# SonyCSLParis/vqcpc-bach

Measured on AMD Instinct MI355X. Metric: encoder-train windows/sec (Bach 4-voice, seq=256), higher is better.
Workload: dtype f32

## Files before the change

### include/vqcpc.h

```cpp
#ifndef VQCPC_H
#define VQCPC_H

#include <stdint.h>

#ifdef __cplusplus
extern "C" {
#endif

#define VQCPC_ABI_VERSION 2

#define VQCPC_OK 0
#define VQCPC_EINVAL (-1)
#define VQCPC_ELAUNCH (-2)
#define VQCPC_EWORKSPACE (-3)

int vqcpc_abi_version(void);
const char* vqcpc_last_error(void);
int vqcpc_clear_runtime_error(void);

int vqcpc_dropout_mask(float* mask, int64_t n, float p, uint64_t seed, void* stream);

int vqcpc_check_tokens(const int64_t* tokens, int64_t n, int n_voices, const int32_t* limits, int64_t* clamped, int32_t* flag,
                       void* stream);

// ... 147 lines not shown
                            const float* mean, const float* rstd, float* d_s, float* d_r, float* d_gamma, float* d_beta,
                            int64_t M, int d, float drop_p, uint64_t seed, void* workspace, int64_t workspace_bytes,
                            void* stream);
int vqcpc_add_layernorm_fwd_b16(const float* x, int64_t ldx, const float* r, const float* gamma, const float* beta, float* y,
                                void* y_bf16, float* mean, float* rstd, int64_t M, int d, float eps, float drop_p,
                                uint64_t seed, void* stream);
int vqcpc_add_layernorm_bwd_b16(const float* dy, const float* x, int64_t ldx, const float* r, const float* gamma,
                                const float* mean, const float* rstd, float* d_s, float* d_r, void* d_r_bf16, float* d_gamma,
                                float* d_beta, int64_t M, int d, float drop_p, uint64_t seed, void* workspace,
                                int64_t workspace_bytes, void* stream);
int vqcpc_layernorm_fwd_xb16(const void* x_bf16, int64_t ldx, const float* gamma, const float* beta, float* y, void* y_bf16,
                             float* mean, float* rstd, int64_t M, int d, float eps, void* stream);
int vqcpc_layernorm_bwd_xb16(const float* dy, const void* x_bf16, int64_t ldx, const float* gamma, const float* mean,
                             const float* rstd, float* d_s, void* d_s_bf16, float* d_r, void* d_r_bf16, float* d_gamma,
                             float* d_beta, int64_t M, int d, float drop_p, uint64_t seed, void* workspace,
                             int64_t workspace_bytes, void* stream);
int vqcpc_layernorm_bwd_b16io(const void* dy_bf16, const void* x_bf16, int64_t ldx, const float* gamma, const float* mean,
                              const float* rstd, float* d_s, void* d_s_bf16, float* d_r, void* d_r_bf16, float* d_gamma,
                              float* d_beta, int64_t M, int d, float drop_p, uint64_t seed, void* workspace,
                              int64_t workspace_bytes, void* stream);
int vqcpc_add_layernorm_bwd_partials(int64_t M, int d, int has_r);
int vqcpc_reduce_grouped(int n, const void* const* ws, const int64_t* stride, const int* nsplit, void* const* out,
                         const int64_t* count, int accumulate, void* stream);

int vqcpc_vq_fwd(const float* z, const float* codebooks, int64_t R, int ncb, int K, int dsub, float beta, int squared,
                 int assign, int64_t* idx, float* zq_sg, float* loss, void* stream);
int64_t vqcpc_vq_bwd_workspace(int64_t R, int ncb, int K, int dsub);
int vqcpc_vq_bwd(const float* z, const float* codebooks, const int64_t* idx, const float* g_zq, const float* g_loss,
                 int64_t R, int ncb, int K, int dsub, float beta, int squared, float* d_z, float* d_codebooks,
                 void* workspace, int64_t workspace_bytes, void* stream);

int64_t vqcpc_vq_ema_stats_workspace(int64_t R, int ncb, int K, int dsub);
int vqcpc_vq_ema_stats(const float* z, const int64_t* idx, int64_t R, int ncb, int K, int dsub, float* stats, void* workspace,
                       int64_t workspace_bytes, void* stream);
int vqcpc_vq_commit_bwd(const float* z, const float* codebooks, const int64_t* idx, const float* g_zq, const float* g_loss,
                        int64_t R, int ncb, int K, int dsub, float beta, int squared, float* d_z, void* stream);
int vqcpc_vq_ema_update(const float* stats, float* cluster_size, float* ema_sum, float* codebooks, int ncb, int K, int dsub,
                        float g, float h, float eps, void* stream);

int vqcpc_vq_restart_candidates(const float* z, int64_t R, int ncb, int K, int dsub, uint64_t seed, uint64_t step,
                                const uint64_t* step_dev, int rank, int world, float* cand, void* stream);
int vqcpc_vq_ema_restart(const float* cand, float* cluster_size, float* ema_sum, float* codebooks, int ncb, int K, int dsub,
                         float thr, int32_t* restarts, void* stream);

int vqcpc_dropout_selu_fwd(const float* h, float* out, int64_t n, float drop_p, uint64_t seed, void* stream);
int vqcpc_dropout_selu_bwd(const float* h, const float* g_out, float* g_h, int64_t n, float drop_p, uint64_t seed,
// ... 231 lines not shown
```

### vqcpc_bach_amd/csrc/common.h

```cpp
#pragma once
#include <stdlib.h>
#include <hip/hip_runtime.h>
#include <stdint.h>
#include <stdio.h>

#include "../../include/vqcpc.h"

namespace vq {

void set_error(const char* fmt, ...);

#define VQ_REQUIRE(cond, ...)                   \
    do {                                        \
        if (!(cond)) {                          \
            vq::set_error(__VA_ARGS__);         \
            return VQCPC_EINVAL;                \
        }                                       \
    } while (0)

#define VQ_CHECK_LAUNCH(name)                                                        \
    do {                                                                             \
        hipError_t e_ = hipGetLastError();                                           \
        if (e_ != hipSuccess) {                                                      \
            vq::set_error("%s: launch failed: %s", name, hipGetErrorString(e_));     \
// ... 43 lines not shown
__device__ __forceinline__ uint32_t rng_u24(uint64_t seed, uint64_t idx) {
    const uint64_t se = rng_seed_eff(seed);
    return rng_u24_from_x0(rng_x0(se, static_cast<uint32_t>(idx)), static_cast<uint32_t>(se >> 32));
}
__host__ __device__ __forceinline__ uint32_t drop_threshold(float p) { return static_cast<uint32_t>(p * 16777216.0f); }
__device__ __forceinline__ float drop_scale(uint64_t seed, uint64_t idx, uint32_t thr, float inv_keep) {
    if (thr == 0) return 1.0f;
    return rng_u24(seed, idx) >= thr ? inv_keep : 0.0f;
}

__device__ __forceinline__ float wave_sum(float v) {
#pragma unroll
    for (int o = 32; o > 0; o >>= 1) v += __shfl_xor(v, o, 64);
    return v;
}
__device__ __forceinline__ float wave_max(float v) {
#pragma unroll
    for (int o = 32; o > 0; o >>= 1) v = fmaxf(v, __shfl_xor(v, o, 64));
    return v;
}

int launch_reduce_splits(const float* ws, int64_t stride, int nsplit, float* out, int64_t count, int accumulate,
                         hipStream_t stream);
int launch_reduce_splits2(const float* ws, int64_t stride, int nsplit, float* out, int64_t count, const float* ws2,
                          int64_t stride2, float* out2, int64_t count2, int accumulate, hipStream_t stream);

#ifdef __HIPCC__
typedef float vq_f32x2_t __attribute__((ext_vector_type(2)));
typedef __bf16 vq_bf16x2_t __attribute__((ext_vector_type(2)));
__device__ __forceinline__ uint32_t bf16x2_rn(float e0, float e1) {
    const vq_f32x2_t v = {e0, e1};
    return __builtin_bit_cast(uint32_t, __builtin_convertvector(v, vq_bf16x2_t));
}
__device__ __forceinline__ void store4_out(float* __restrict__ base, int64_t off, float a, float b, float c, float d, int out16) {
    if (out16)
        *reinterpret_cast<uint2*>(reinterpret_cast<unsigned short*>(base) + off) = make_uint2(bf16x2_rn(a, b), bf16x2_rn(c, d));
    else
        *reinterpret_cast<float4*>(base + off) = make_float4(a, b, c, d);
}
__device__ __forceinline__ void store1_out(float* __restrict__ base, int64_t off, float a, int out16) {
    if (out16) reinterpret_cast<unsigned short*>(base)[off] = (unsigned short)(bf16x2_rn(a, 0.0f) & 0xFFFFu);
    else base[off] = a;
}
#endif

int64_t relattn16_bwd_workspace(int64_t n_blocks, int H, int hd);
// ... 8 lines not shown
```

### vqcpc_bach_amd/csrc/relattn.hip

```cpp
#include "common.h"
#include "relattn_forms.h"
#include <stdlib.h>

namespace vq {

constexpr int kAttThreads = 256;
constexpr int kPad = 4;

template <int L, int HD>
struct AttCfg {
    static constexpr int LPP = 4 * L;
    static constexpr int PPW = 64 / LPP;
    static constexpr int SLOTS = 4 * PPW;
    static constexpr int JPL = L / 4;
    static constexpr int CPL = HD / 4;
    static constexpr int RS = HD + kPad;
    static constexpr int NE = 2 * L - 1;
    static constexpr int FWD_FLOATS = (3 * L + NE) * RS + L * (L + 1);
    static constexpr int BWD_FLOATS = (4 * L + NE) * RS + 2 * L * (L + 1);
};

template <int L, int HD>
__device__ __forceinline__ void stage_rows(float* dst, const float* __restrict__ src, int64_t ld, int sl, float mul,
                                           const int64_t* __restrict__ tok = nullptr) {
// ... 317 lines not shown
#pragma unroll
                            for (int c4 = 0; c4 < C::CPL / 4; ++c4) {
                                const float4 q = *reinterpret_cast<const float4*>(Qs + ii * C::RS + jg * C::CPL + c4 * 4);
                                de[a][c4 * 4 + 0] += ds * q.x; de[a][c4 * 4 + 1] += ds * q.y;
                                de[a][c4 * 4 + 2] += ds * q.z; de[a][c4 * 4 + 3] += ds * q.w;
                            }
                        }
                    }
                }
            }
        }
    }
    float* dst = ws + ((((int64_t)blockIdx.x * NS + nsub) * H + h) * C::NE) * HD;
#pragma unroll
    for (int a = 0; a < 2; ++a) {
        const int r = i + a * L;
        if (r < C::NE) {
#pragma unroll
            for (int c = 0; c < C::CPL; ++c) dst[r * HD + jg * C::CPL + c] = de[a][c];
        }
    }
}

__global__ __launch_bounds__(256) void relattn_de_split(const float* __restrict__ tot, int H, int L, int HD,
                                                        float* __restrict__ d_e1, float* __restrict__ d_e2) {
    const int NE = 2 * L - 1;
    const int o = blockIdx.x * blockDim.x + threadIdx.x;
    if (o >= H * NE * HD) return;
    const int c = o % HD, r = (o / HD) % NE, h = o / (HD * NE);
    const float acc = tot[o];
    if (r < L) d_e1[((int64_t)h * L + r) * HD + c] = acc;
    else d_e2[((int64_t)h * L + (r - L + 1)) * HD + c] = acc;
    if (r == 0) d_e2[((int64_t)h * L) * HD + c] = 0.0f;
}

static int att_blocks_per_wg(int64_t n_blocks, int slots, int H) {
    const int ns = std::max(1, slots / H);
    int64_t b = ceil_div(n_blocks, 2048);
    b = round_up(std::max<int64_t>(b, ns), ns);
    return (int)b;
}

template <int L, int HD>
static int launch_fwd(const float* qkv, int64_t ldq, const float* e1, const float* e2, float* ctx, int64_t ldo,
                      float* probs, int64_t n_blocks, int H, float drop_p, uint64_t seed, hipStream_t s,
                      const int64_t* tokens, int o16) {
    using C = AttCfg<L, HD>;
    const size_t lds = (size_t)C::SLOTS * C::FWD_FLOATS * sizeof(float);
    auto kern = relattn_fwd_kernel<L, HD>;
    if (lds > 64 * 1024) (void)hipFuncSetAttribute((const void*)kern, hipFuncAttributeMaxDynamicSharedMemorySize, (int)lds);
    int64_t grid = std::min<int64_t>(ceil_div(n_blocks * H, C::SLOTS), 2048);
    int gcd = H, rem = C::SLOTS;
    while (rem) { const int t = gcd % rem; gcd = rem; rem = t; }
    const int64_t unit = H / gcd;
    grid = ceil_div(grid, unit) * unit;
    hipLaunchKernelGGL(kern, dim3((unsigned)grid), dim3(kAttThreads), lds, s, qkv, ldq, e1, e2, ctx, ldo, probs, n_blocks,
                       H, 1.0f / sqrtf((float)HD), drop_threshold(drop_p), 1.0f / (1.0f - drop_p), seed, tokens, o16);
    VQ_CHECK_LAUNCH("relattn_fwd");
    return VQCPC_OK;
}

template <int L, int HD>
static int launch_bwd(const float* d_ctx, int64_t ldo, const float* qkv, int64_t ldq, const float* probs, const float* e1,
                      const float* e2, float* d_qkv, int64_t ldg, float* d_e1, float* d_e2, int64_t n_blocks, int H,
                      float drop_p, uint64_t seed, float* ws, hipStream_t s, const int64_t* tokens, int g16) {
    using C = AttCfg<L, HD>;
    const size_t lds = (size_t)C::SLOTS * C::BWD_FLOATS * sizeof(float);
    auto kern = relattn_bwd_kernel<L, HD>;
    if (lds > 64 * 1024) (void)hipFuncSetAttribute((const void*)kern, hipFuncAttributeMaxDynamicSharedMemorySize, (int)lds);
    const int bpw = att_blocks_per_wg(n_blocks, C::SLOTS, H);
    const int chunks = (int)ceil_div(n_blocks, bpw);
    const int gy = C::SLOTS >= H ? 1 : H / C::SLOTS;
    const int NS = C::SLOTS >= H ? C::SLOTS / H : 1;
    hipLaunchKernelGGL(kern, dim3(chunks, gy), dim3(kAttThreads), lds, s, d_ctx, ldo, qkv, ldq, probs, e1, e2, d_qkv, ldg,
                       ws, n_blocks, H, bpw, 1.0f / sqrtf((float)HD), drop_threshold(drop_p), 1.0f / (1.0f - drop_p), seed, tokens, g16);
    VQ_CHECK_LAUNCH("relattn_bwd");
    const int total = H * C::NE * HD;
    float* tot = ws + (int64_t)chunks * NS * total;
    int rc = launch_reduce_splits(ws, total, chunks * NS, tot, total, 0, s);
    if (rc) return rc;
    hipLaunchKernelGGL(relattn_de_split, dim3(ceil_div(total, 256)), dim3(256), 0, s, tot, H, L, HD, d_e1, d_e2);
    VQ_CHECK_LAUNCH("relattn_de_split");
    return VQCPC_OK;
}

static int g_force_general = 0;
static bool use_mfma16(int L, int H, int hd) { return att_mfma16_ok(L, H, hd); }
static bool att_supported(int L, int H, int hd) { return !g_force_general && att_lds_ok(L, H, hd); }

static int finish_de16(float* ws, int nsplit, int H, int hd, float* d_e1, float* d_e2, hipStream_t s) {
    const int total = H * 31 * hd;
    float* tot = ws + (int64_t)nsplit * total;
    int rc = launch_reduce_splits(ws, total, nsplit, tot, total, 0, s);
    if (rc) return rc;
    hipLaunchKernelGGL(relattn_de_split, dim3(ceil_div(total, 256)), dim3(256), 0, s, tot, H, 16, hd, d_e1, d_e2);
    VQ_CHECK_LAUNCH("relattn_de_split");
    return VQCPC_OK;
}

static AttRoute route_of(const AttEntry& e, int L, int H, int hd, const int64_t* tokens, const void* qkv, const void* e1,
                         const void* e2, const void* out, const void* d_ctx = nullptr, const void* ws = nullptr) {
    const unsigned aligned = (aligned16(qkv) ? P_QKV : 0) | (aligned16(e1) ? P_E1 : 0) | (aligned16(e2) ? P_E2 : 0) |
                             (aligned16(out) ? P_OUT : 0) | (aligned16(d_ctx) ? P_DCTX : 0) | (aligned16(ws) ? P_WS : 0);
    return att_route(e, L, H, hd, g_force_general != 0, aligned, tokens != nullptr);
}

static int self_fwd(int family, const void* qkv, int64_t ldq, const int64_t* tokens, const float* e1, const float* e2, void* ctx,
                    int64_t ldo, float* probs, int64_t n_blocks, int L, int H, int hd, float drop_p, uint64_t seed, void* stream) {
    const AttEntry& e = kAttEntries[2 * family];
    if (n_blocks == 0) return VQCPC_OK;
    VQ_REQUIRE(qkv && e1 && e2 && ctx && probs, "%s: null pointer", e.name);
    VQ_REQUIRE(ldq % (e.io & IN16 ? 8 : 4) == 0 && ldo % 4 == 0 && ldq >= 3 * H * hd && ldo >= H * hd && n_blocks >= 0,
               "%s: bad strides", e.name);
    VQ_REQUIRE(drop_p >= 0.f && drop_p < 1.f, "%s: bad dropout probability", e.name);
    const AttRoute r = route_of(e, L, H, hd, tokens, qkv, e1, e2, ctx);
    VQ_REQUIRE(r.kernel != ATT_REFUSED, "%s: %s L=%d H=%d hd=%d", e.name, r.why, L, H, hd);
    hipStream_t s = (hipStream_t)stream;
    if (r.kernel == ATT_STRIP) {
        VQ_REQUIRE(n_blocks * H * (int64_t)((L + 31) / 32) < (1ll << 31), "%s: too many strips", e.name);
        const float* q = (const float*)qkv;
// ... 145 lines not shown
```

### vqcpc_bach_amd/csrc/relattn_sub.hip

```cpp
#include "common.h"

namespace vq {

constexpr int kSubPad = 4;

template <int L, int HD, int F>
struct SubCfg {
    static constexpr int LQ = L / F;
    static constexpr int LPP = 4 * LQ;
    static constexpr int PPW = 64 / LPP;
    static constexpr int JPL = L / 4;
    static constexpr int CPL = HD / 4;
    static constexpr int RS = HD + kSubPad;
    static constexpr int NE = 2 * L - 1;
    static constexpr int NER = (NE + LQ - 1) / LQ;
    static constexpr int FWD_FLOATS = (LQ + 2 * L + NE) * RS + LQ * (L + 1);
    static constexpr int BWD_FLOATS = (2 * LQ + 2 * L + NE) * RS + 2 * LQ * (L + 1);
};

template <int ROWS, int HD, int LPP>
__device__ __forceinline__ void sub_stage(float* dst, const float* __restrict__ src, int64_t ld, int sl, float mul) {
    constexpr int RS = HD + kSubPad, V = HD / 4;
    for (int e = sl; e < ROWS * V; e += LPP) {
        const int row = e / V, c4 = e % V;
// ... 619 lines not shown
#pragma unroll
                            for (int c4 = 0; c4 < C::C4 / 4; ++c4) {
                                const float4 qq = *reinterpret_cast<const float4*>(Qs + ii * C::RS + cgE * C::C4 + c4 * 4);
                                de[a][c4 * 4 + 0] += ds * qq.x; de[a][c4 * 4 + 1] += ds * qq.y;
                                de[a][c4 * 4 + 2] += ds * qq.z; de[a][c4 * 4 + 3] += ds * qq.w;
                            }
                        }
                    }
                }
            }
        }
    }
    float* dst = ws + ((((int64_t)blockIdx.x * NS + nsub) * H + h) * C::NE) * HD;
#pragma unroll
    for (int a = 0; a < 2; ++a) {
        const int r = rr + 16 * a;
        if (r < C::NE) {
#pragma unroll
            for (int c = 0; c < C::C4; ++c) dst[r * HD + cgE * C::C4 + c] = de[a][c];
        }
    }
}

__global__ __launch_bounds__(256) void relattn_sub_de_split(const float* __restrict__ tot, int H, int L, int HD,
                                                            float* __restrict__ d_e1, float* __restrict__ d_e2) {
    const int NE = 2 * L - 1;
    const int o = blockIdx.x * blockDim.x + threadIdx.x;
    if (o >= H * NE * HD) return;
    const int c = o % HD, r = (o / HD) % NE, h = o / (HD * NE);
    const float acc = tot[o];
    if (r < L) d_e1[((int64_t)h * L + r) * HD + c] = acc;
    else d_e2[((int64_t)h * L + (r - L + 1)) * HD + c] = acc;
    if (r == 0) d_e2[((int64_t)h * L) * HD + c] = 0.0f;
}

static int sub_blocks_per_wg(int64_t n_blocks, int ppw, int H) {
    const int ns = std::max(1, ppw / H);
    int64_t b = ceil_div(n_blocks, 4096);
    return (int)round_up(std::max<int64_t>(b, ns), ns);
}

static bool sub_supported(int L, int F, int H, int hd) {
    if (!((L == 16 || L == 4) && F == 4)) return false;
    if (!(hd == 16 || hd == 32 || hd == 64)) return false;
    const int ppw = 64 / (4 * (L / F));
    return H >= 1 && ((ppw % H) == 0 || (H % ppw) == 0);
}

template <int L, int HD, int F>
static int sub_launch_fwd(const float* q, int64_t ldq, const float* kv, int64_t ldkv, const float* e1, const float* e2,
                          float* ctx, int64_t ldo, float* probs, int64_t n_blocks, int H, float drop_p, uint64_t seed,
                          hipStream_t s, int b16) {
    using C = SubCfg<L, HD, F>;
    const size_t lds = (size_t)C::PPW * C::FWD_FLOATS * sizeof(float);
    auto kern = relattn_sub_fwd_kernel<L, HD, F>;
    if (lds > 64 * 1024) (void)hipFuncSetAttribute((const void*)kern, hipFuncAttributeMaxDynamicSharedMemorySize, (int)lds);
    int64_t grid = std::min<int64_t>(ceil_div(n_blocks * H, C::PPW), 8192);
    int gcd = H, rem = C::PPW;
// ... 5 lines not shown
    VQ_CHECK_LAUNCH("relattn_sub_fwd");
    return VQCPC_OK;
}

template <int L, int HD, int F>
static int sub_launch_bwd(const float* d_ctx, int64_t ldo, const float* q, int64_t ldq, const float* kv, int64_t ldkv,
                          const float* probs, const float* e1, const float* e2, float* d_q, int64_t ldgq, float* d_kv,
                          int64_t ldgkv, float* d_e1, float* d_e2, int64_t n_blocks, int H, float drop_p, uint64_t seed,
                          float* ws, hipStream_t s, int b16) {
    using C = SubCfg<L, HD, F>;
    const size_t lds = (size_t)C::PPW * C::BWD_FLOATS * sizeof(float);
    auto kern = relattn_sub_bwd_kernel<L, HD, F>;
    if (lds > 64 * 1024) (void)hipFuncSetAttribute((const void*)kern, hipFuncAttributeMaxDynamicSharedMemorySize, (int)lds);
    const int bpw = sub_blocks_per_wg(n_blocks, C::PPW, H);
    const int chunks = (int)ceil_div(n_blocks, bpw);
    const int gy = C::PPW >= H ? 1 : H / C::PPW;
    const int NS = C::PPW >= H ? C::PPW / H : 1;
    hipLaunchKernelGGL(kern, dim3(chunks, gy), dim3(64), lds, s, d_ctx, ldo, q, ldq, kv, ldkv, probs, e1, e2, d_q, ldgq,
                       d_kv, ldgkv, ws, n_blocks, H, bpw, 1.0f / sqrtf((float)HD), drop_threshold(drop_p),
                       1.0f / (1.0f - drop_p), seed, b16);
    VQ_CHECK_LAUNCH("relattn_sub_bwd");
    const int total = H * C::NE * HD;
    float* tot = ws + (int64_t)chunks * NS * total;
    int rc = launch_reduce_splits(ws, total, chunks * NS, tot, total, 0, s);
    if (rc) return rc;
    hipLaunchKernelGGL(relattn_sub_de_split, dim3(ceil_div(total, 256)), dim3(256), 0, s, tot, H, L, HD, d_e1, d_e2);
    VQ_CHECK_LAUNCH("relattn_sub_de_split");
    return VQCPC_OK;
}

static int sub16_blocks_per_wg(int64_t n_blocks, int H) {
    const int ns = std::max(1, 4 / H);
    int64_t b = ceil_div(n_blocks, 4096);
    return (int)round_up(std::max<int64_t>(b, ns), ns);
}

template <int HD>
static int sub16_launch_fwd(const float* q, int64_t ldq, const float* kv, int64_t ldkv, const float* e1, const float* e2,
                            float* ctx, int64_t ldo, float* probs, int64_t n_blocks, int H, float drop_p, uint64_t seed,
                            hipStream_t s, int b16) {
    using C = Sub16<HD>;
    const size_t lds = (size_t)4 * C::FWD_FLOATS * sizeof(float);
    auto kern = relattn_sub16_fwd_kernel<HD>;
    if (lds > 64 * 1024) (void)hipFuncSetAttribute((const void*)kern, hipFuncAttributeMaxDynamicSharedMemorySize, (int)lds);
    int64_t grid = std::min<int64_t>(ceil_div(n_blocks * H, 4), 2048);
    int gcd = H, rem = 4;
    while (rem) { const int t = gcd % rem; gcd = rem; rem = t; }
    const int64_t unit = H / gcd;
    grid = ceil_div(grid, unit) * unit;
    hipLaunchKernelGGL(kern, dim3((unsigned)grid), dim3(256), lds, s, q, ldq, kv, ldkv, e1, e2, ctx, ldo, probs, n_blocks, H,
                       1.0f / sqrtf((float)HD), drop_threshold(drop_p), 1.0f / (1.0f - drop_p), seed, b16);
    VQ_CHECK_LAUNCH("relattn_sub16_fwd");
    return VQCPC_OK;
}

template <int HD>
static int sub16_launch_bwd(const float* d_ctx, int64_t ldo, const float* q, int64_t ldq, const float* kv, int64_t ldkv,
                            const float* probs, const float* e1, const float* e2, float* d_q, int64_t ldgq, float* d_kv,
                            int64_t ldgkv, float* d_e1, float* d_e2, int64_t n_blocks, int H, float drop_p, uint64_t seed,
                            float* ws, hipStream_t s, int b16) {
    using C = Sub16<HD>;
    const size_t lds = (size_t)4 * C::BWD_FLOATS * sizeof(float);
    auto kern = relattn_sub16_bwd_kernel<HD>;
    if (lds > 64 * 1024) (void)hipFuncSetAttribute((const void*)kern, hipFuncAttributeMaxDynamicSharedMemorySize, (int)lds);
    const int bpw = sub16_blocks_per_wg(n_blocks, H);
    const int chunks = (int)ceil_div(n_blocks, bpw);
    const int gy = 4 >= H ? 1 : H / 4;
    const int NS = 4 >= H ? 4 / H : 1;
    hipLaunchKernelGGL(kern, dim3(chunks, gy), dim3(256), lds, s, d_ctx, ldo, q, ldq, kv, ldkv, probs, e1, e2, d_q, ldgq, d_kv,
                       ldgkv, ws, n_blocks, H, bpw, 1.0f / sqrtf((float)HD), drop_threshold(drop_p), 1.0f / (1.0f - drop_p),
                       seed, b16);
    VQ_CHECK_LAUNCH("relattn_sub16_bwd");
    const int total = H * C::NE * HD;
    float* tot = ws + (int64_t)chunks * NS * total;
    int rc = launch_reduce_splits(ws, total, chunks * NS, tot, total, 0, s);
    if (rc) return rc;
    hipLaunchKernelGGL(relattn_sub_de_split, dim3(ceil_div(total, 256)), dim3(256), 0, s, tot, H, 16, HD, d_e1, d_e2);
    VQ_CHECK_LAUNCH("relattn_sub_de_split");
    return VQCPC_OK;
}

}

using namespace vq;

#define VQ_SUB_DISPATCH(CALL)                        \
    if (L == 16 && hd == 16) return CALL(16, 16, 4); \
    if (L == 16 && hd == 32) return CALL(16, 32, 4); \
    if (L == 16 && hd == 64) return CALL(16, 64, 4); \
    if (L == 4 && hd == 16) return CALL(4, 16, 4);   \
    if (L == 4 && hd == 32) return CALL(4, 32, 4);   \
    if (L == 4 && hd == 64) return CALL(4, 64, 4);

extern "C" {

static int sub_fwd_impl(const float* q, int64_t ldq, const float* kv, int64_t ldkv, const float* e1, const float* e2,
                        float* ctx, int64_t ldo, float* probs, int64_t n_blocks, int L, int F, int H, int hd, float drop_p,
                        uint64_t seed, void* stream, int b16) {
    if (n_blocks == 0) return VQCPC_OK;
    VQ_REQUIRE(q && kv && e1 && e2 && ctx && probs, "relattn_sub_fwd: null pointer");
    VQ_REQUIRE(sub_supported(L, F, H, hd), "relattn_sub_fwd: unsupported L=%d F=%d H=%d hd=%d", L, F, H, hd);
    VQ_REQUIRE(ldq % 4 == 0 && ldkv % 4 == 0 && ldo % 4 == 0 && ldq >= H * hd && ldkv >= 2 * H * hd && ldo >= H * hd &&
// ... 95 lines not shown
```

### vqcpc_bach_amd/csrc/util.hip

```cpp
#include <stdarg.h>

#include <algorithm>

#include "common.h"

namespace vq {

static thread_local char g_err[512] = "";

void set_error(const char* fmt, ...) {
    va_list ap;
    va_start(ap, fmt);
    vsnprintf(g_err, sizeof(g_err), fmt, ap);
    va_end(ap);
}

constexpr int kRedCols = 64, kRedGroups = 16;

__global__ __launch_bounds__(kRedCols * kRedGroups) void reduce_splits_kernel(const float* __restrict__ ws,
                                                                              int64_t stride, int nsplit,
                                                                              float* __restrict__ out, int64_t count,
                                                                              const float* __restrict__ ws2, int64_t stride2,
                                                                              float* __restrict__ out2, int64_t count2,
                                                                              int accumulate) {
    __shared__ float part[kRedGroups][kRedCols];
    const int tx = threadIdx.x % kRedCols, ty = threadIdx.x / kRedCols;
    int64_t col = (int64_t)blockIdx.x * kRedCols + tx;
    const int64_t first = (count + kRedCols - 1) / kRedCols * kRedCols;
    if (col >= first) {
        col -= first;
        ws = ws2;
        stride = stride2;
        out = out2;
        count = count2;
    }
    float acc = 0.0f;
    if (col < count) {
        int s = ty;
        for (; s + 3 * kRedGroups < nsplit; s += 4 * kRedGroups) {
            const float a = ws[(int64_t)s * stride + col];
            const float b = ws[(int64_t)(s + kRedGroups) * stride + col];
            const float c = ws[(int64_t)(s + 2 * kRedGroups) * stride + col];
            const float d = ws[(int64_t)(s + 3 * kRedGroups) * stride + col];
            acc = ((acc + a) + b) + (c + d);
        }
        for (; s < nsplit; s += kRedGroups) acc += ws[(int64_t)s * stride + col];
    }
    part[ty][tx] = acc;
    __syncthreads();
    if (ty == 0 && col < count) {
        float tot = accumulate ? out[col] : 0.0f;
#pragma unroll
        for (int g = 0; g < kRedGroups; ++g) tot += part[g][tx];
        out[col] = tot;
    }
}

constexpr int kRedVecThreads = 256;

__global__ __launch_bounds__(kRedVecThreads) void reduce_splits_vec_kernel(const float* __restrict__ ws, int64_t stride,
                                                                          int nsplit, float* __restrict__ out, int64_t count,
                                                                          const float* __restrict__ ws2, int64_t stride2,
                                                                          float* __restrict__ out2, int64_t count2,
                                                                          int accumulate) {
    int64_t q = (int64_t)blockIdx.x * kRedVecThreads + threadIdx.x;
    const int64_t first = (count / 4 + kRedVecThreads - 1) / kRedVecThreads * kRedVecThreads;
    if (q >= first) {
        q -= first;
        ws = ws2;
        stride = stride2;
        out = out2;
        count = count2;
    }
    if (q * 4 >= count) return;
    const float4* p = reinterpret_cast<const float4*>(ws) + q;
    const int64_t st4 = stride / 4;
    float4 acc = make_float4(0.f, 0.f, 0.f, 0.f);
// ... 43 lines not shown
    return VQCPC_OK;
}

constexpr int kRedMany = 32;
struct RedManyArgs {
    const float* ws[kRedMany];
    float* out[kRedMany];
    int stride[kRedMany], nsplit[kRedMany], count[kRedMany];
    int blk_begin[kRedMany + 1];
    int n, accumulate;
};

__global__ __launch_bounds__(kRedCols * kRedGroups) void reduce_many_kernel(const RedManyArgs g) {
    __shared__ float part[kRedGroups][kRedCols];
    const int b = (int)blockIdx.x;
    int p = 0;
    for (int i = 1; i < g.n; ++i) p += (b >= g.blk_begin[i]) ? 1 : 0;
    p = __builtin_amdgcn_readfirstlane(p);
    const float* __restrict__ ws = g.ws[p];
    const int64_t stride = g.stride[p];
    const int nsplit = g.nsplit[p], count = g.count[p];
    const int tx = threadIdx.x % kRedCols, ty = threadIdx.x / kRedCols;
    const int col = (b - g.blk_begin[p]) * kRedCols + tx;
    float acc = 0.0f;
    if (col < count) {
        int s = ty;
        for (; s + 3 * kRedGroups < nsplit; s += 4 * kRedGroups) {
            const float a = ws[(int64_t)s * stride + col];
            const float b2 = ws[(int64_t)(s + kRedGroups) * stride + col];
            const float c = ws[(int64_t)(s + 2 * kRedGroups) * stride + col];
            const float d = ws[(int64_t)(s + 3 * kRedGroups) * stride + col];
            acc = ((acc + a) + b2) + (c + d);
        }
        for (; s < nsplit; s += kRedGroups) acc += ws[(int64_t)s * stride + col];
    }
    part[ty][tx] = acc;
    __syncthreads();
    if (ty == 0 && col < count) {
        float* out = g.out[p];
        float tot = g.accumulate ? out[col] : 0.0f;
#pragma unroll
        for (int q = 0; q < kRedGroups; ++q) tot += part[q][tx];
        out[col] = tot;
    }
}

__global__ __launch_bounds__(kRedVecThreads) void reduce_many_vec_kernel(const RedManyArgs g) {
    const int b = (int)blockIdx.x;
    int p = 0;
    for (int i = 1; i < g.n; ++i) p += (b >= g.blk_begin[i]) ? 1 : 0;
    p = __builtin_amdgcn_readfirstlane(p);
    const int64_t q = (int64_t)(b - g.blk_begin[p]) * kRedVecThreads + threadIdx.x;
    if (q * 4 >= g.count[p]) return;
    const float4* ptr = reinterpret_cast<const float4*>(g.ws[p]) + q;
    const int64_t st4 = g.stride[p] / 4;
    const int nsplit = g.nsplit[p];
    float4 acc = make_float4(0.f, 0.f, 0.f, 0.f);
#define RV_ADD(X, Y) make_float4(X.x + Y.x, X.y + Y.y, X.z + Y.z, X.w + Y.w)
    int s = 0;
// ... 1 lines not shown
        const float4 v0 = ptr[(s + 0) * st4], v1 = ptr[(s + 1) * st4], v2 = ptr[(s + 2) * st4], v3 = ptr[(s + 3) * st4];
        const float4 v4 = ptr[(s + 4) * st4], v5 = ptr[(s + 5) * st4], v6 = ptr[(s + 6) * st4], v7 = ptr[(s + 7) * st4];
        const float4 a = RV_ADD(v0, v1), bb = RV_ADD(v2, v3), c = RV_ADD(v4, v5), d = RV_ADD(v6, v7);
        const float4 ab = RV_ADD(a, bb), cd = RV_ADD(c, d);
        const float4 t = RV_ADD(ab, cd);
        acc = RV_ADD(acc, t);
    }
    for (; s < nsplit; ++s) {
        const float4 v = ptr[s * st4];
        acc = RV_ADD(acc, v);
    }
    float4* o = reinterpret_cast<float4*>(g.out[p]) + q;
    if (g.accumulate) {
        const float4 prev = *o;
        acc = RV_ADD(prev, acc);
    }
#undef RV_ADD
    *o = acc;
}

int launch_reduce_splits(const float* ws, int64_t stride, int nsplit, float* out, int64_t count, int accumulate,
                         hipStream_t stream) {
    return launch_reduce_splits2(ws, stride, nsplit, out, count, nullptr, 0, nullptr, 0, accumulate, stream);
}

__global__ __launch_bounds__(256) void dropout_mask_kernel(float* mask, int64_t n, uint32_t thr, uint64_t seed) {
    int64_t i = (int64_t)blockIdx.x * blockDim.x + threadIdx.x;
    const int64_t step = (int64_t)gridDim.x * blockDim.x;
    for (; i < n; i += step) mask[i] = (thr == 0 || rng_u24(seed, (uint64_t)i) >= thr) ? 1.0f : 0.0f;
}

__global__ __launch_bounds__(256) void transpose_kernel(const float* __restrict__ in, float* __restrict__ out, int R,
                                                        int C) {
    __shared__ float tile[32][33];
    const int tx = threadIdx.x & 31, ty = threadIdx.x >> 5;
    const int c0 = blockIdx.x * 32, r0 = blockIdx.y * 32;
#pragma unroll
    for (int k = 0; k < 4; ++k) {
        int r = r0 + ty + k * 8, c = c0 + tx;
        if (r < R && c < C) tile[ty + k * 8][tx] = in[(int64_t)r * C + c];
    }
    __syncthreads();
#pragma unroll
    for (int k = 0; k < 4; ++k) {
        int c = c0 + ty + k * 8, r = r0 + tx;
        if (r < R && c < C) out[(int64_t)c * R + r] = tile[tx][ty + k * 8];
// ... 535 lines not shown
            if (dup) break;
            g.ws[c] = (const float*)ws[i];
            g.out[c] = (float*)out[i];
            g.stride[c] = (int)stride[i];
            g.nsplit[c] = nsplit[i];
            g.count[c] = (int)count[i];
            g.blk_begin[c] = rb;
            rb += (int)ceil_div(count[i] / 4, (int64_t)kRedVecThreads);
            ++c;
            ++i;
        }
        for (int j = c; j <= kRedMany; ++j) g.blk_begin[j] = rb;
        for (int j = c; j < kRedMany; ++j) {
            g.ws[j] = nullptr; g.out[j] = nullptr; g.stride[j] = g.nsplit[j] = g.count[j] = 0;
        }
        g.n = c;
        g.accumulate = accumulate;
        hipLaunchKernelGGL(reduce_many_vec_kernel, dim3((unsigned)rb), dim3(kRedVecThreads), 0, s, g);
        VQ_CHECK_LAUNCH("reduce_grouped_vec");
    }
    return VQCPC_OK;
}

int vqcpc_reduce_grouped(int n, const void* const* ws, const int64_t* stride, const int* nsplit, void* const* out,
                         const int64_t* count, int accumulate, void* stream) {
    if (n == 0) return VQCPC_OK;
    VQ_REQUIRE(n > 0 && ws && stride && nsplit && out && count, "reduce_grouped: null pointer");
    for (int i = 0; i < n; ++i)
        VQ_REQUIRE(ws[i] && out[i] && nsplit[i] >= 1 && count[i] >= 1 && stride[i] >= count[i] && stride[i] < (1ll << 31) &&
                       count[i] < (1ll << 31),
                   "reduce_grouped: bad segment %d", i);
    hipStream_t s = (hipStream_t)stream;
    int i = 0;
    while (i < n) {
        RedManyArgs g;
        int c = 0, rb = 0;
        while (i < n && c < kRedMany) {
            bool dup = false;
            for (int j = 0; j < c; ++j) dup = dup || g.out[j] == (float*)out[i];
            if (dup) break;
            g.ws[c] = (const float*)ws[i];
            g.out[c] = (float*)out[i];
            g.stride[c] = (int)stride[i];
            g.nsplit[c] = nsplit[i];
            g.count[c] = (int)count[i];
            g.blk_begin[c] = rb;
// ... 18 lines not shown
```

### vqcpc_bach_amd/hip.py

```python
import ctypes
import os

import torch

_HERE = os.path.dirname(os.path.abspath(__file__))
LIB_PATH = os.path.join(_HERE, 'libvqcpc_hip.so')
ABI_VERSION = 2

_lib = None

c_i64, c_int, c_f32, c_u64, c_ptr = ctypes.c_int64, ctypes.c_int, ctypes.c_float, ctypes.c_uint64, ctypes.c_void_p

SIGNATURES = {
    'vqcpc_abi_version': (c_int, []),
    'vqcpc_last_error': (ctypes.c_char_p, []),
    'vqcpc_clear_runtime_error': (c_int, []),
    'vqcpc_dropout_mask': (c_int, [c_ptr, c_i64, c_f32, c_u64, c_ptr]),
    'vqcpc_check_tokens': (c_int, [c_ptr, c_i64, c_int, c_ptr, c_ptr, c_ptr, c_ptr]),
    'vqcpc_embed_pos_fwd': (c_int, [c_ptr, c_i64, c_int, c_int, c_ptr, c_int, c_int, c_ptr, c_ptr, c_int, c_ptr, c_ptr]),
    'vqcpc_embed_pos_bwd_workspace': (c_i64, [c_i64, c_int, c_int, c_int, c_int, c_int]),
    'vqcpc_embed_pos_bwd': (c_int, [c_ptr, c_i64, c_int, c_int, c_int, c_int, c_int, c_ptr, c_ptr, c_ptr, c_ptr, c_ptr,
                                    c_i64, c_ptr]),
    'vqcpc_block_table_gather': (c_int, [c_ptr, c_ptr, c_ptr, c_i64, c_int, c_int, c_int, c_ptr]),
    'vqcpc_block_table_segsum_workspace': (c_i64, [c_i64, c_int, c_int, c_int]),
# ... 89 lines not shown
    'vqcpc_relattn_x_bwd_workspace': (c_i64, [c_i64, c_int, c_int, c_int, c_int]),
    'vqcpc_relattn_x_bwd': (c_int, [c_ptr, c_i64, c_ptr, c_i64, c_ptr, c_i64, c_ptr, c_i64, c_ptr, c_ptr, c_ptr, c_ptr, c_i64,
                                    c_ptr, c_i64, c_ptr, c_i64, c_ptr, c_ptr, c_i64, c_int, c_int, c_int, c_int, c_int, c_f32,
                                    c_u64, c_ptr, c_i64, c_ptr]),
    'vqcpc_embedding_bwd': (c_int, [c_ptr, c_i64, c_ptr, c_ptr, c_ptr, c_i64, c_i64, c_int, c_ptr]),
    'vqcpc_product_gather': (c_int, [c_ptr, c_ptr, c_ptr, c_i64, c_ptr, c_int, c_ptr, c_i64, c_i64, c_int, c_int, c_int, c_int,
                                     c_ptr]),
    'vqcpc_product_gather_bwd': (c_int, [c_ptr, c_i64, c_ptr, c_ptr, c_ptr, c_ptr, c_i64, c_i64, c_int, c_int, c_int, c_int, c_ptr]),
    'vqcpc_add_layernorm_fwd': (c_int, [c_ptr, c_i64, c_ptr, c_ptr, c_ptr, c_ptr, c_ptr, c_ptr, c_i64, c_int, c_f32,
                                        c_f32, c_u64, c_ptr]),
    'vqcpc_add_layernorm_fwd_b16': (c_int, [c_ptr, c_i64, c_ptr, c_ptr, c_ptr, c_ptr, c_ptr, c_ptr, c_ptr, c_i64, c_int, c_f32,
                                            c_f32, c_u64, c_ptr]),
    'vqcpc_add_layernorm_bwd_b16': (c_int, [c_ptr, c_ptr, c_i64, c_ptr, c_ptr, c_ptr, c_ptr, c_ptr, c_ptr, c_ptr, c_ptr, c_ptr,
                                            c_i64, c_int, c_f32, c_u64, c_ptr, c_i64, c_ptr]),
    'vqcpc_layernorm_fwd_xb16': (c_int, [c_ptr, c_i64, c_ptr, c_ptr, c_ptr, c_ptr, c_ptr, c_ptr, c_i64, c_int, c_f32, c_ptr]),
    'vqcpc_layernorm_bwd_xb16': (c_int, [c_ptr, c_ptr, c_i64, c_ptr, c_ptr, c_ptr, c_ptr, c_ptr, c_ptr, c_ptr, c_ptr, c_ptr, c_i64,
                                         c_int, c_f32, c_u64, c_ptr, c_i64, c_ptr]),
    'vqcpc_layernorm_bwd_b16io': (c_int, [c_ptr, c_ptr, c_i64, c_ptr, c_ptr, c_ptr, c_ptr, c_ptr, c_ptr, c_ptr, c_ptr, c_ptr, c_i64,
                                          c_int, c_f32, c_u64, c_ptr, c_i64, c_ptr]),
    'vqcpc_add_layernorm_bwd_workspace': (c_i64, [c_i64, c_int]),
    'vqcpc_add_layernorm_bwd_partials': (c_int, [c_i64, c_int, c_int]),
    'vqcpc_reduce_grouped': (c_int, [c_int, c_ptr, c_ptr, c_ptr, c_ptr, c_ptr, c_int, c_ptr]),
    'vqcpc_reduce_grouped_vec': (c_int, [c_int, c_ptr, c_ptr, c_ptr, c_ptr, c_ptr, c_int, c_ptr]),
    'vqcpc_gemm_tn_deferred_splits': (c_int, [c_i64, c_int, c_int]),
    'vqcpc_gemm_tn_bf16_deferred_splits': (c_int, [c_i64, c_int, c_int]),
    'vqcpc_add_layernorm_bwd': (c_int, [c_ptr, c_ptr, c_i64, c_ptr, c_ptr, c_ptr, c_ptr, c_ptr, c_ptr, c_ptr, c_ptr,
                                        c_i64, c_int, c_f32, c_u64, c_ptr, c_i64, c_ptr]),
    'vqcpc_vq_fwd': (c_int, [c_ptr, c_ptr, c_i64, c_int, c_int, c_int, c_f32, c_int, c_int, c_ptr, c_ptr, c_ptr, c_ptr]),
    'vqcpc_vq_bwd_workspace': (c_i64, [c_i64, c_int, c_int, c_int]),
    'vqcpc_vq_bwd': (c_int, [c_ptr, c_ptr, c_ptr, c_ptr, c_ptr, c_i64, c_int, c_int, c_int, c_f32, c_int, c_ptr, c_ptr,
                             c_ptr, c_i64, c_ptr]),
    'vqcpc_vq_ema_stats_workspace': (c_i64, [c_i64, c_int, c_int, c_int]),
    'vqcpc_vq_ema_stats': (c_int, [c_ptr, c_ptr, c_i64, c_int, c_int, c_int, c_ptr, c_ptr, c_i64, c_ptr]),
    'vqcpc_vq_commit_bwd': (c_int, [c_ptr, c_ptr, c_ptr, c_ptr, c_ptr, c_i64, c_int, c_int, c_int, c_f32, c_int, c_ptr, c_ptr]),
    'vqcpc_vq_ema_update': (c_int, [c_ptr, c_ptr, c_ptr, c_ptr, c_int, c_int, c_int, c_f32, c_f32, c_f32, c_ptr]),
    'vqcpc_vq_restart_candidates': (c_int, [c_ptr, c_i64, c_int, c_int, c_int, c_u64, c_u64, c_ptr, c_int, c_int, c_ptr, c_ptr]),
    'vqcpc_vq_ema_restart': (c_int, [c_ptr, c_ptr, c_ptr, c_ptr, c_int, c_int, c_int, c_f32, c_ptr, c_ptr]),
    'vqcpc_dropout_selu_fwd': (c_int, [c_ptr, c_ptr, c_i64, c_f32, c_u64, c_ptr]),
    'vqcpc_dropout_selu_bwd': (c_int, [c_ptr, c_ptr, c_ptr, c_i64, c_f32, c_u64, c_ptr]),
    'vqcpc_nce_fwd': (c_int, [c_ptr, c_ptr, c_ptr, c_ptr, c_int, c_int, c_int, c_int, c_int, c_ptr, c_ptr, c_ptr, c_ptr,
                              c_ptr]),
    'vqcpc_nce_bwd_workspace': (c_i64, [c_int, c_int, c_int, c_int, c_int]),
    'vqcpc_nce_bwd': (c_int, [c_ptr, c_ptr, c_ptr, c_ptr, c_ptr, c_ptr, c_ptr, c_int, c_int, c_int, c_int, c_int, c_ptr,
                              c_ptr, c_ptr, c_ptr, c_ptr, c_i64, c_ptr]),
    'vqcpc_sumsq_workspace': (c_i64, [c_i64]),
    'vqcpc_sumsq': (c_int, [c_ptr, c_i64, c_f32, c_ptr, c_ptr, c_i64, c_ptr]),
# ... 230 lines not shown
```

Baseline: 11750.

## Fuse relative-embedding split reduction with d_e1/d_e2 scatter and add two-phase path

Replaces the reduce-splits kernel plus separate de_split scatter with a shared launcher. By default it fuses the split reduction and the d_e1/d_e2 scatter into one kernel. When there are many splits and few output tiles it instead runs a two-phase reduction (per-group partial sums written in place into ws, then a combine-and-scatter kernel) to expose more parallelism. The inner reduction loop also gains a deeper unrolled prefetch of 32 loads per iteration to hide memory latency. The cost is a changed summation order and in-place overwriting of the workspace rows.

```diff
diff --git a/include/vqcpc.h b/include/vqcpc.h
--- a/include/vqcpc.h
+++ b/include/vqcpc.h
@@ -193,6 +193,8 @@
 int vqcpc_add_layernorm_bwd_partials(int64_t M, int d, int has_r);
 int vqcpc_reduce_grouped(int n, const void* const* ws, const int64_t* stride, const int* nsplit, void* const* out,
                          const int64_t* count, int accumulate, void* stream);
+int vqcpc_reduce_relemb(float* ws, int64_t stride, int nsplit, float* scratch, int H, int L, int hd, float* d_e1,
+                        float* d_e2, void* stream);
 
 int vqcpc_vq_fwd(const float* z, const float* codebooks, int64_t R, int ncb, int K, int dsub, float beta, int squared,
                  int assign, int64_t* idx, float* zq_sg, float* loss, void* stream);
diff --git a/vqcpc_bach_amd/csrc/common.h b/vqcpc_bach_amd/csrc/common.h
--- a/vqcpc_bach_amd/csrc/common.h
+++ b/vqcpc_bach_amd/csrc/common.h
@@ -89,6 +89,8 @@
 
 int launch_reduce_splits(const float* ws, int64_t stride, int nsplit, float* out, int64_t count, int accumulate,
                          hipStream_t stream);
+int launch_reduce_splits_de(float* ws, int64_t stride, int nsplit, float* tot, int H, int L, int HD, float* d_e1, float* d_e2,
+                            hipStream_t stream);
 int launch_reduce_splits2(const float* ws, int64_t stride, int nsplit, float* out, int64_t count, const float* ws2,
                           int64_t stride2, float* out2, int64_t count2, int accumulate, hipStream_t stream);
 
diff --git a/vqcpc_bach_amd/csrc/relattn.hip b/vqcpc_bach_amd/csrc/relattn.hip
--- a/vqcpc_bach_amd/csrc/relattn.hip
+++ b/vqcpc_bach_amd/csrc/relattn.hip
@@ -363,18 +363,6 @@
     }
 }
 
-__global__ __launch_bounds__(256) void relattn_de_split(const float* __restrict__ tot, int H, int L, int HD,
-                                                        float* __restrict__ d_e1, float* __restrict__ d_e2) {
-    const int NE = 2 * L - 1;
-    const int o = blockIdx.x * blockDim.x + threadIdx.x;
-    if (o >= H * NE * HD) return;
-    const int c = o % HD, r = (o / HD) % NE, h = o / (HD * NE);
-    const float acc = tot[o];
-    if (r < L) d_e1[((int64_t)h * L + r) * HD + c] = acc;
-    else d_e2[((int64_t)h * L + (r - L + 1)) * HD + c] = acc;
-    if (r == 0) d_e2[((int64_t)h * L) * HD + c] = 0.0f;
-}
-
 static int att_blocks_per_wg(int64_t n_blocks, int slots, int H) {
     const int ns = std::max(1, slots / H);
     int64_t b = ceil_div(n_blocks, 2048);
@@ -418,11 +406,7 @@
     VQ_CHECK_LAUNCH("relattn_bwd");
     const int total = H * C::NE * HD;
     float* tot = ws + (int64_t)chunks * NS * total;
-    int rc = launch_reduce_splits(ws, total, chunks * NS, tot, total, 0, s);
-    if (rc) return rc;
-    hipLaunchKernelGGL(relattn_de_split, dim3(ceil_div(total, 256)), dim3(256), 0, s, tot, H, L, HD, d_e1, d_e2);
-    VQ_CHECK_LAUNCH("relattn_de_split");
-    return VQCPC_OK;
+    return launch_reduce_splits_de(ws, total, chunks * NS, tot, H, L, HD, d_e1, d_e2, s);
 }
 
 static int g_force_general = 0;
@@ -432,11 +416,7 @@
 static int finish_de16(float* ws, int nsplit, int H, int hd, float* d_e1, float* d_e2, hipStream_t s) {
     const int total = H * 31 * hd;
     float* tot = ws + (int64_t)nsplit * total;
-    int rc = launch_reduce_splits(ws, total, nsplit, tot, total, 0, s);
-    if (rc) return rc;
-    hipLaunchKernelGGL(relattn_de_split, dim3(ceil_div(total, 256)), dim3(256), 0, s, tot, H, 16, hd, d_e1, d_e2);
-    VQ_CHECK_LAUNCH("relattn_de_split");
-    return VQCPC_OK;
+    return launch_reduce_splits_de(ws, total, nsplit, tot, H, 16, hd, d_e1, d_e2, s);
 }
 
 static AttRoute route_of(const AttEntry& e, int L, int H, int hd, const int64_t* tokens, const void* qkv, const void* e1,
diff --git a/vqcpc_bach_amd/csrc/relattn_sub.hip b/vqcpc_bach_amd/csrc/relattn_sub.hip
--- a/vqcpc_bach_amd/csrc/relattn_sub.hip
+++ b/vqcpc_bach_amd/csrc/relattn_sub.hip
@@ -665,18 +665,6 @@
     }
 }
 
-__global__ __launch_bounds__(256) void relattn_sub_de_split(const float* __restrict__ tot, int H, int L, int HD,
-                                                            float* __restrict__ d_e1, float* __restrict__ d_e2) {
-    const int NE = 2 * L - 1;
-    const int o = blockIdx.x * blockDim.x + threadIdx.x;
-    if (o >= H * NE * HD) return;
-    const int c = o % HD, r = (o / HD) % NE, h = o / (HD * NE);
-    const float acc = tot[o];
-    if (r < L) d_e1[((int64_t)h * L + r) * HD + c] = acc;
-    else d_e2[((int64_t)h * L + (r - L + 1)) * HD + c] = acc;
-    if (r == 0) d_e2[((int64_t)h * L) * HD + c] = 0.0f;
-}
-
 static int sub_blocks_per_wg(int64_t n_blocks, int ppw, int H) {
     const int ns = std::max(1, ppw / H);
     int64_t b = ceil_div(n_blocks, 4096);
@@ -728,11 +716,7 @@
     VQ_CHECK_LAUNCH("relattn_sub_bwd");
     const int total = H * C::NE * HD;
     float* tot = ws + (int64_t)chunks * NS * total;
-    int rc = launch_reduce_splits(ws, total, chunks * NS, tot, total, 0, s);
-    if (rc) return rc;
-    hipLaunchKernelGGL(relattn_sub_de_split, dim3(ceil_div(total, 256)), dim3(256), 0, s, tot, H, L, HD, d_e1, d_e2);
-    VQ_CHECK_LAUNCH("relattn_sub_de_split");
-    return VQCPC_OK;
+    return launch_reduce_splits_de(ws, total, chunks * NS, tot, H, L, HD, d_e1, d_e2, s);
 }
 
 static int sub16_blocks_per_wg(int64_t n_blocks, int H) {
@@ -779,11 +763,7 @@
     VQ_CHECK_LAUNCH("relattn_sub16_bwd");
     const int total = H * C::NE * HD;
     float* tot = ws + (int64_t)chunks * NS * total;
-    int rc = launch_reduce_splits(ws, total, chunks * NS, tot, total, 0, s);
-    if (rc) return rc;
-    hipLaunchKernelGGL(relattn_sub_de_split, dim3(ceil_div(total, 256)), dim3(256), 0, s, tot, H, 16, HD, d_e1, d_e2);
-    VQ_CHECK_LAUNCH("relattn_sub_de_split");
-    return VQCPC_OK;
+    return launch_reduce_splits_de(ws, total, chunks * NS, tot, H, 16, HD, d_e1, d_e2, s);
 }
 
 }
diff --git a/vqcpc_bach_amd/csrc/util.hip b/vqcpc_bach_amd/csrc/util.hip
--- a/vqcpc_bach_amd/csrc/util.hip
+++ b/vqcpc_bach_amd/csrc/util.hip
@@ -16,6 +16,30 @@
 }
 
 constexpr int kRedCols = 64, kRedGroups = 16;
+
+constexpr int kRedAhead = 8;
+
+__device__ __forceinline__ float red_group_sum(const float* ws, int64_t stride, int nsplit, int64_t col, int ty) {
+    float acc = 0.0f;
+    int s = ty;
+    for (; s + (4 * kRedAhead - 1) * kRedGroups < nsplit; s += 4 * kRedAhead * kRedGroups) {
+        const float* p = ws + (int64_t)s * stride + col;
+        float v[4 * kRedAhead];
+#pragma unroll
+        for (int u = 0; u < 4 * kRedAhead; ++u) v[u] = p[(int64_t)u * kRedGroups * stride];
+#pragma unroll
+        for (int u = 0; u < kRedAhead; ++u) acc = ((acc + v[4 * u]) + v[4 * u + 1]) + (v[4 * u + 2] + v[4 * u + 3]);
+    }
+    for (; s + 3 * kRedGroups < nsplit; s += 4 * kRedGroups) {
+        const float a = ws[(int64_t)s * stride + col];
+        const float b = ws[(int64_t)(s + kRedGroups) * stride + col];
+        const float c = ws[(int64_t)(s + 2 * kRedGroups) * stride + col];
+        const float d = ws[(int64_t)(s + 3 * kRedGroups) * stride + col];
+        acc = ((acc + a) + b) + (c + d);
+    }
+    for (; s < nsplit; s += kRedGroups) acc += ws[(int64_t)s * stride + col];
+    return acc;
+}
 
 __global__ __launch_bounds__(kRedCols * kRedGroups) void reduce_splits_kernel(const float* __restrict__ ws,
                                                                               int64_t stride, int nsplit,
@@ -34,25 +58,34 @@
         out = out2;
         count = count2;
     }
-    float acc = 0.0f;
-    if (col < count) {
-        int s = ty;
-        for (; s + 3 * kRedGroups < nsplit; s += 4 * kRedGroups) {
-            const float a = ws[(int64_t)s * stride + col];
-            const float b = ws[(int64_t)(s + kRedGroups) * stride + col];
-            const float c = ws[(int64_t)(s + 2 * kRedGroups) * stride + col];
-            const float d = ws[(int64_t)(s + 3 * kRedGroups) * stride + col];
-            acc = ((acc + a) + b) + (c + d);
-        }
-        for (; s < nsplit; s += kRedGroups) acc += ws[(int64_t)s * stride + col];
-    }
-    part[ty][tx] = acc;
+    part[ty][tx] = col < count ? red_group_sum(ws, stride, nsplit, col, ty) : 0.0f;
     __syncthreads();
     if (ty == 0 && col < count) {
         float tot = accumulate ? out[col] : 0.0f;
 #pragma unroll
         for (int g = 0; g < kRedGroups; ++g) tot += part[g][tx];
         out[col] = tot;
+    }
+}
+
+__global__ __launch_bounds__(kRedCols * kRedGroups) void reduce_splits_de_kernel(const float* __restrict__ ws, int64_t stride,
+                                                                                 int nsplit, int H, int L, int HD,
+                                                                                 float* __restrict__ d_e1,
+                                                                                 float* __restrict__ d_e2) {
+    __shared__ float part[kRedGroups][kRedCols];
+    const int tx = threadIdx.x % kRedCols, ty = threadIdx.x / kRedCols;
+    const int NE = 2 * L - 1, count = H * NE * HD;
+    const int col = (int)blockIdx.x * kRedCols + tx;
+    part[ty][tx] = col < count ? red_group_sum(ws, stride, nsplit, col, ty) : 0.0f;
+    __syncthreads();
+    if (ty == 0 && col < count) {
+        float tot = 0.0f;
+#pragma unroll
+        for (int g = 0; g < kRedGroups; ++g) tot += part[g][tx];
+        const int c = col % HD, r = (col / HD) % NE, h = col / (HD * NE);
+        if (r < L) d_e1[((int64_t)h * L + r) * HD + c] = tot;
+        else d_e2[((int64_t)h * L + (r - L + 1)) * HD + c] = tot;
+        if (r == 0) d_e2[((int64_t)h * L) * HD + c] = 0.0f;
     }
 }
 
@@ -142,19 +175,7 @@
     const int nsplit = g.nsplit[p], count = g.count[p];
     const int tx = threadIdx.x % kRedCols, ty = threadIdx.x / kRedCols;
     const int col = (b - g.blk_begin[p]) * kRedCols + tx;
-    float acc = 0.0f;
-    if (col < count) {
-        int s = ty;
-        for (; s + 3 * kRedGroups < nsplit; s += 4 * kRedGroups) {
-            const float a = ws[(int64_t)s * stride + col];
-            const float b2 = ws[(int64_t)(s + kRedGroups) * stride + col];
-            const float c = ws[(int64_t)(s + 2 * kRedGroups) * stride + col];
-            const float d = ws[(int64_t)(s + 3 * kRedGroups) * stride + col];
-            acc = ((acc + a) + b2) + (c + d);
-        }
-        for (; s < nsplit; s += kRedGroups) acc += ws[(int64_t)s * stride + col];
-    }
-    part[ty][tx] = acc;
+    part[ty][tx] = col < count ? red_group_sum(ws, stride, nsplit, col, ty) : 0.0f;
     __syncthreads();
     if (ty == 0 && col < count) {
         float* out = g.out[p];
@@ -202,6 +223,69 @@
 int launch_reduce_splits(const float* ws, int64_t stride, int nsplit, float* out, int64_t count, int accumulate,
                          hipStream_t stream) {
     return launch_reduce_splits2(ws, stride, nsplit, out, count, nullptr, 0, nullptr, 0, accumulate, stream);
+}
+
+__global__ __launch_bounds__(256) void relemb_de_split_kernel(const float* __restrict__ tot, int H, int L, int HD,
+                                                              float* __restrict__ d_e1, float* __restrict__ d_e2) {
+    const int NE = 2 * L - 1;
+    const int o = blockIdx.x * blockDim.x + threadIdx.x;
+    if (o >= H * NE * HD) return;
+    const int c = o % HD, r = (o / HD) % NE, h = o / (HD * NE);
+    const float acc = tot[o];
+    if (r < L) d_e1[((int64_t)h * L + r) * HD + c] = acc;
+    else d_e2[((int64_t)h * L + (r - L + 1)) * HD + c] = acc;
+    if (r == 0) d_e2[((int64_t)h * L) * HD + c] = 0.0f;
+}
+
+__global__ __launch_bounds__(kRedCols) void reduce_group_rows_kernel(float* ws, int64_t stride, int nsplit, int count) {
+    const int col = (int)blockIdx.x * kRedCols + threadIdx.x, g = (int)blockIdx.y;
+    if (col >= count || g >= nsplit) return;
+    const float acc = red_group_sum(ws, stride, nsplit, col, g);
+    ws[(int64_t)g * stride + col] = acc;
+}
+
+__global__ __launch_bounds__(256) void relemb_combine_split_kernel(const float* __restrict__ ws, int64_t stride, int nsplit, int H,
+                                                                   int L, int HD, float* __restrict__ d_e1,
+                                                                   float* __restrict__ d_e2) {
+    const int NE = 2 * L - 1;
+    const int o = blockIdx.x * blockDim.x + threadIdx.x;
+    if (o >= H * NE * HD) return;
+    float tot = 0.0f;
+#pragma unroll
+    for (int g = 0; g < kRedGroups; ++g) tot += g < nsplit ? ws[(int64_t)g * stride + o] : 0.0f;
+    const int c = o % HD, r = (o / HD) % NE, h = o / (HD * NE);
+    if (r < L) d_e1[((int64_t)h * L + r) * HD + c] = tot;
+    else d_e2[((int64_t)h * L + (r - L + 1)) * HD + c] = tot;
+    if (r == 0) d_e2[((int64_t)h * L) * HD + c] = 0.0f;
+}
+
+constexpr int kRedTwoPhaseSplits = 512, kRedTwoPhaseMaxTiles = 64;
+
+int launch_reduce_splits_de(float* ws, int64_t stride, int nsplit, float* tot, int H, int L, int HD, float* d_e1, float* d_e2,
+                            hipStream_t stream) {
+    const int64_t count = (int64_t)H * (2 * L - 1) * HD;
+    VQ_REQUIRE(ws && tot && d_e1 && d_e2 && H >= 1 && L >= 1 && HD >= 1 && nsplit >= 0 && count < (1 << 30) && stride >= count,
+               "reduce_splits_de: bad arguments");
+    if (nsplit >= kRedTwoPhaseSplits && ceil_div(count, kRedCols) <= kRedTwoPhaseMaxTiles) {
+        hipLaunchKernelGGL(reduce_group_rows_kernel, dim3((unsigned)ceil_div(count, kRedCols), kRedGroups), dim3(kRedCols), 0, stream,
+                           ws, stride, nsplit, (int)count);
+        VQ_CHECK_LAUNCH("reduce_group_rows");
+        hipLaunchKernelGGL(relemb_combine_split_kernel, dim3((unsigned)ceil_div(count, 256)), dim3(256), 0, stream, ws, stride,
+                           nsplit, H, L, HD, d_e1, d_e2);
+        VQ_CHECK_LAUNCH("relemb_combine_split");
+        return VQCPC_OK;
+    }
+    if (count >= (1 << 16) && nsplit <= 64 && reduce_vec_ok(ws, stride, tot, count)) {
+        if (int rc = launch_reduce_splits(ws, stride, nsplit, tot, count, 0, stream)) return rc;
+        hipLaunchKernelGGL(relemb_de_split_kernel, dim3((unsigned)ceil_div(count, 256)), dim3(256), 0, stream, tot, H, L, HD, d_e1,
+                           d_e2);
+        VQ_CHECK_LAUNCH("relemb_de_split");
+        return VQCPC_OK;
+    }
+    hipLaunchKernelGGL(reduce_splits_de_kernel, dim3((unsigned)ceil_div(count, kRedCols)), dim3(kRedCols * kRedGroups), 0, stream,
+                       ws, stride, nsplit, H, L, HD, d_e1, d_e2);
+    VQ_CHECK_LAUNCH("reduce_splits_de");
+    return VQCPC_OK;
 }
 
 __global__ __launch_bounds__(256) void dropout_mask_kernel(float* mask, int64_t n, uint32_t thr, uint64_t seed) {
@@ -783,6 +867,13 @@
     return VQCPC_OK;
 }
 
+int vqcpc_reduce_relemb(float* ws, int64_t stride, int nsplit, float* scratch, int H, int L, int hd, float* d_e1,
+                        float* d_e2, void* stream) {
+    VQ_REQUIRE(H >= 1 && L >= 1 && hd >= 1 && nsplit >= 1 && stride >= (int64_t)H * (2 * L - 1) * hd && stride < (1ll << 31),
+               "reduce_relemb: bad shape (H=%d L=%d hd=%d nsplit=%d)", H, L, hd, nsplit);
+    return launch_reduce_splits_de(ws, stride, nsplit, scratch, H, L, hd, d_e1, d_e2, (hipStream_t)stream);
+}
+
 int vqcpc_reduce_grouped(int n, const void* const* ws, const int64_t* stride, const int* nsplit, void* const* out,
                          const int64_t* count, int accumulate, void* stream) {
     if (n == 0) return VQCPC_OK;
diff --git a/vqcpc_bach_amd/hip.py b/vqcpc_bach_amd/hip.py
--- a/vqcpc_bach_amd/hip.py
+++ b/vqcpc_bach_amd/hip.py
@@ -135,6 +135,7 @@
     'vqcpc_add_layernorm_bwd_partials': (c_int, [c_i64, c_int, c_int]),
     'vqcpc_reduce_grouped': (c_int, [c_int, c_ptr, c_ptr, c_ptr, c_ptr, c_ptr, c_int, c_ptr]),
     'vqcpc_reduce_grouped_vec': (c_int, [c_int, c_ptr, c_ptr, c_ptr, c_ptr, c_ptr, c_int, c_ptr]),
+    'vqcpc_reduce_relemb': (c_int, [c_ptr, c_i64, c_int, c_ptr, c_int, c_int, c_int, c_ptr, c_ptr, c_ptr]),
     'vqcpc_gemm_tn_deferred_splits': (c_int, [c_i64, c_int, c_int]),
     'vqcpc_gemm_tn_bf16_deferred_splits': (c_int, [c_i64, c_int, c_int]),
     'vqcpc_add_layernorm_bwd': (c_int, [c_ptr, c_ptr, c_i64, c_ptr, c_ptr, c_ptr, c_ptr, c_ptr, c_ptr, c_ptr, c_ptr,
```

Result: no change. 11780, median of 6 (+0.2%).
